# ryogrid/anime-illust-image-searcher

Hardware: AMD Instinct MI355X
Metric: images/sec tagged (ViT fwd) (higher is better)
Workload: dtype f16; 1 GPU; wd-tagger ViT-B/16 448px 16-bit-operand forward + sigmoid + MCut tag selection, batch 64 per GPU, u8 NHWC images resident in HBM (BASELINE.json configs[1]); batch_per_gpu=64, image=448x448x3 u8, classes=10861, parallelism=single GPU

## Files before the change

### anime-illust-image-searcher_amd/csrc/tags.hip

```cpp
#include <vector>

#include "common.h"
#include "rank_util.h"

using namespace hipts;

struct hipts_tagsel {
    int device = 0;
    int C = 0, max_batch = 0;
    int ng = 0, nc = 0, npad = 0;
    DevBuf gidx, cidx;
    DevBuf ws_probs, ws_counts, ws_ids, ws_thresh;
    int ws_row_cap = 0;
};

namespace {

__device__ void bitonic_desc(uint64_t* keys, int npad) {
    for (int size = 2; size <= npad; size <<= 1) {
        for (int stride = size >> 1; stride > 0; stride >>= 1) {
            for (int t = threadIdx.x; t < (npad >> 1); t += blockDim.x) {
                const int lo = ((t / stride) * stride * 2) + (t % stride);
                const int hi = lo + stride;
                const bool desc = ((lo & size) == 0);
                const uint64_t a = keys[lo], b = keys[hi];
                if ((a > b) != desc) {
                    keys[lo] = b;
                    keys[hi] = a;
                }
            }
            __syncthreads();
        }
    }
}

__device__ void select_category(const float* __restrict__ probs, const int32_t* __restrict__ idx, int n, int npad,
                                bool mcut, double thresh_in, bool floor015, uint64_t* keys, double* sh_d, int* sh_i,
                                int32_t* __restrict__ ids_out, int cap, int* count_out, double* thresh_out) {
    const int tid = threadIdx.x, nthr = blockDim.x;
    for (int i = tid; i < npad; i += nthr) {
        uint64_t k = 0;
        if (i < n) k = ((uint64_t)float_order_key_canon(probs[idx[i]]) << 32) | (uint64_t)(0xffffffffu - (uint32_t)i);
        keys[i] = k;
    }
    __syncthreads();
    bitonic_desc(keys, npad);
    double thresh = thresh_in;
    if (mcut && n >= 2) {
        double best = -INFINITY;
        int besti = 0x7fffffff;
        for (int i = tid; i < n - 1; i += nthr) {
            const double a = (double)float_from_key((uint32_t)(keys[i] >> 32));
            const double b = (double)float_from_key((uint32_t)(keys[i + 1] >> 32));
            const double dif = a - b;
            if (dif > best) {
                best = dif;
                besti = i;
            }
        }
        for (int o = 32; o >= 1; o >>= 1) {
            const double ob = __shfl_xor(best, o);
            const int oi = __shfl_xor(besti, o);
            if (ob > best || (ob == best && oi < besti)) {
                best = ob;
                besti = oi;
            }
        }
        if ((tid & 63) == 0) {
            sh_d[tid >> 6] = best;
            sh_i[tid >> 6] = besti;
        }
        __syncthreads();
        if (tid == 0) {
            double b = sh_d[0];
            int bi = sh_i[0];
            for (int w = 1; w < (nthr >> 6); ++w)
                if (sh_d[w] > b || (sh_d[w] == b && sh_i[w] < bi)) {
                    b = sh_d[w];
                    bi = sh_i[w];
                }
            const double a0 = (double)float_from_key((uint32_t)(keys[bi] >> 32));
            const double a1 = (double)float_from_key((uint32_t)(keys[bi + 1] >> 32));
            double t = (a0 + a1) / 2;
            if (floor015 && !(t > 0.15)) t = 0.15;
            sh_d[16] = t;
        }
        __syncthreads();
        thresh = sh_d[16];
        __syncthreads();
    } else if (mcut && floor015 && !(thresh > 0.15)) {
        thresh = 0.15;
    }
    int cnt = 0;
    for (int i = tid; i < n; i += nthr)
        if ((double)float_from_key((uint32_t)(keys[i] >> 32)) > thresh) ++cnt;
    for (int o = 32; o >= 1; o >>= 1) cnt += __shfl_xor(cnt, o);
    if ((tid & 63) == 0) sh_i[tid >> 6] = cnt;
    __syncthreads();
    if (tid == 0) {
        int c = 0;
        for (int w = 0; w < (nthr >> 6); ++w) c += sh_i[w];
        sh_i[16] = c;
    }
    __syncthreads();
    const int total = sh_i[16];
    for (int i = tid; i < total && i < cap; i += nthr)
        ids_out[i] = idx[0xffffffffu - (uint32_t)(keys[i] & 0xffffffffu)];
    if (tid == 0) {
        *count_out = total;
        *thresh_out = thresh;
    }
    __syncthreads();
}

__global__ __launch_bounds__(1024) void tagsel_kernel(const float* __restrict__ probs, int C, const int32_t* __restrict__ gidx,
                                                      int ng, const int32_t* __restrict__ cidx, int nc, int npad,
                                                      double g_thresh, int g_mcut, double c_thresh, int c_mcut,
                                                      int32_t* __restrict__ counts, int counts_stride,
                                                      int32_t* __restrict__ ids, int ids_stride, int row_cap,
                                                      double* __restrict__ thresh) {
    extern __shared__ __attribute__((aligned(16))) uint64_t keys[];
    __shared__ double sh_d[17];
    __shared__ int sh_i[17];
    __shared__ int sh_cnt[2];
    __shared__ double sh_thr[2];
    const int b = blockIdx.x;
    const float* __restrict__ row = probs + (int64_t)b * C;
    int32_t* __restrict__ out = ids + (int64_t)b * ids_stride;
    int npg = 64;
    while (npg < ng) npg <<= 1;
    int npc = 64;
    while (npc < nc) npc <<= 1;
    select_category(row, gidx, ng, npg, g_mcut != 0, g_thresh, false, keys, sh_d, sh_i, out, row_cap, &sh_cnt[0], &sh_thr[0]);
    const int n_g = sh_cnt[0];
    const int used = n_g < row_cap ? n_g : row_cap;
    select_category(row, cidx, nc, npc, c_mcut != 0, c_thresh, true, keys, sh_d, sh_i, out + used, row_cap - used, &sh_cnt[1],
                    &sh_thr[1]);
    if (threadIdx.x == 0) {
        counts[(int64_t)b * counts_stride] = sh_cnt[0];
        counts[(int64_t)b * counts_stride + 1] = sh_cnt[1];
        if (thresh) {
            thresh[2 * b] = sh_thr[0];
            thresh[2 * b + 1] = sh_thr[1];
        }
    }
}

}

extern "C" {

int hipts_tagsel_create(const int32_t* category, int num_classes, int device, int max_batch, hipts_tagsel_t** out) {
    HIPTS_REQUIRE(category && out && num_classes >= 1 && max_batch >= 1, "hipts_tagsel_create: bad arguments");
    HIPTS_TRY(use_device(device));
    std::vector<int32_t> g, c;
    for (int i = 0; i < num_classes; ++i) {
        if (category[i] == 0) g.push_back(i);
        else if (category[i] == 4) c.push_back(i);
    }
    int npad = 64;
    while (npad < (int)g.size() || npad < (int)c.size()) npad <<= 1;
    HIPTS_REQUIRE((size_t)npad * 8 <= 144 * 1024, "hipts_tagsel_create: a category with %zu labels does not fit the LDS sort",
                  g.size() > c.size() ? g.size() : c.size());
    auto* h = new hipts_tagsel();
    h->device = device;
    h->C = num_classes;
    h->max_batch = max_batch;
    h->ng = (int)g.size();
    h->nc = (int)c.size();
    h->npad = npad;
    int st;
    if ((st = h->gidx.alloc(g.size() * 4)) || (st = h->cidx.alloc(c.size() * 4)) || (st = upload(h->gidx.p, g.data(), g.size() * 4)) ||
        (st = upload(h->cidx.p, c.data(), c.size() * 4))) {
        delete h;
        return st;
    }
    hipError_t e = hipFuncSetAttribute((const void*)tagsel_kernel, hipFuncAttributeMaxDynamicSharedMemorySize, 144 * 1024);
    if (e != hipSuccess) {
        delete h;
        return set_error(HIPTS_ERR_HIP, "hipFuncSetAttribute failed: %s", hipGetErrorString(e));
    }
    *out = h;
    return HIPTS_OK;
}

int hipts_tagsel_destroy(hipts_tagsel_t* h) {
    if (h) {
        (void)hipSetDevice(h->device);
        delete h;
    }
    return HIPTS_OK;
}

int hipts_tagsel_run(hipts_tagsel_t* h, const float* probs, int probs_memspace, int batch, double general_thresh,
                     int general_mcut, double character_thresh, int character_mcut, int32_t* counts_out, int32_t* ids_out,
                     int row_cap, double* thresh_out, int out_memspace, void* stream) {
    HIPTS_REQUIRE(h && probs && counts_out && ids_out && batch >= 1 && row_cap >= 1, "hipts_tagsel_run: bad arguments");
    HIPTS_TRY(use_device(h->device));
    hipStream_t s = (hipStream_t)stream;
    const float* p_dev = probs;
    if (probs_memspace != HIPTS_DEVICE) {
        HIPTS_TRY(h->ws_probs.reserve((size_t)batch * h->C * 4));
        HIPTS_HIP(hipMemcpyAsync(h->ws_probs.p, probs, (size_t)batch * h->C * 4, hipMemcpyHostToDevice, s));
        p_dev = h->ws_probs.as<float>();
    }
    int32_t* cnt_dev = counts_out;
    int32_t* ids_dev = ids_out;
    double* thr_dev = thresh_out;
    const bool host_out = out_memspace != HIPTS_DEVICE;
    if (host_out || !thresh_out) {
        HIPTS_TRY(h->ws_thresh.reserve((size_t)batch * 16));
        thr_dev = h->ws_thresh.as<double>();
    }
    if (host_out) {
        HIPTS_TRY(h->ws_counts.reserve((size_t)batch * 8));
        HIPTS_TRY(h->ws_ids.reserve((size_t)batch * row_cap * 4));
        cnt_dev = h->ws_counts.as<int32_t>();
        ids_dev = h->ws_ids.as<int32_t>();
    }
    tagsel_kernel<<<batch, 1024, (size_t)h->npad * 8, s>>>(p_dev, h->C, h->gidx.as<int32_t>(), h->ng, h->cidx.as<int32_t>(), h->nc,
                                                           h->npad, general_thresh, general_mcut, character_thresh,
                                                           character_mcut, cnt_dev, 2, ids_dev, row_cap, row_cap, thr_dev);
    HIPTS_LAUNCH_CHECK();
    if (host_out) {
        HIPTS_HIP(hipMemcpyAsync(counts_out, cnt_dev, (size_t)batch * 8, hipMemcpyDeviceToHost, s));
        HIPTS_HIP(hipMemcpyAsync(ids_out, ids_dev, (size_t)batch * row_cap * 4, hipMemcpyDeviceToHost, s));
        if (thresh_out) HIPTS_HIP(hipMemcpyAsync(thresh_out, thr_dev, (size_t)batch * 16, hipMemcpyDeviceToHost, s));
        HIPTS_HIP(hipStreamSynchronize(s));
    }
    return HIPTS_OK;
}

int hipts_tagsel_run_rows(hipts_tagsel_t* h, const float* probs_device, int batch, double general_thresh, int general_mcut,
                          double character_thresh, int character_mcut, int32_t* rows_device, int row_width, void* stream) {
    HIPTS_REQUIRE(h && probs_device && rows_device && batch >= 1 && row_width >= 3, "hipts_tagsel_run_rows: bad arguments");
    HIPTS_TRY(use_device(h->device));
    tagsel_kernel<<<batch, 1024, (size_t)h->npad * 8, (hipStream_t)stream>>>(
        probs_device, h->C, h->gidx.as<int32_t>(), h->ng, h->cidx.as<int32_t>(), h->nc, h->npad, general_thresh, general_mcut,
        character_thresh, character_mcut, rows_device, row_width, rows_device + 2, row_width, row_width - 2, nullptr);
    HIPTS_LAUNCH_CHECK();
    return HIPTS_OK;
}

}
```

### include/hip_tagsearch_debug.h

```cpp
#ifndef HIP_TAGSEARCH_DEBUG_H
#define HIP_TAGSEARCH_DEBUG_H

#include <stddef.h>
#include <stdint.h>

#include "hip_tagsearch.h"

#ifdef __cplusplus
extern "C" {
#endif

int hiptsdbg_gemm_time(int M, int N, int K, int epi, int iters, float* ms_out);
int hiptsdbg_gemm_clock(int M, int N, int K, int epi, int iters, float* ms_out, float* loop_ghz);
int hiptsdbg_gemm_q4_compare(int M, int N, int K, int epi, int f16, int iters, long long* mismatch_out, float* ms_out);
int hiptsdbg_gelu(const float* x_host, int n, int tanh_form, float* y_host);
int hiptsdbg_dwconv7(const uint16_t* in_f16, const float* w, uint16_t* out_f16, int batch, int H, int C, int mode, int iters, float* ms_out);
int hiptsdbg_dwconv7_stamps(unsigned long long* host, int n);
int hiptsdbg_convnext_stream(hipts_convnext_t* h, const float* x_host, int batch, int stage, float* out_host);
int hiptsdbg_swinv2_stream(hipts_swinv2_t* h, const float* x_host, int batch, int stage, float* out_host);
int hiptsdbg_swinv2_window_attention(const float* q, const float* k, const float* v, const float* logit_scale, const float* cpb, int batch,
                                     int heads, int side, int window, int shift, int operand_f16, float* out);
int hiptsdbg_mlp_fused(const uint16_t* xn, const float* w1, const float* w2, float* x, const float* res_scale, const float* gamma, uint16_t* xn_out,
                       int M, int C, float star_s, float star_b, float eps, int iters, float* ms_out, int waves);
int hiptsdbg_mlp_stamps(unsigned long long* host, int n);
int hiptsdbg_mlp_weight_image(const float* w1, const float* w2, int C, uint16_t* out, long long out_halves);
int hiptsdbg_dw_toeplitz(const float* w, int channels, uint32_t* out);
enum { HIPTSDBG_GEMM_V1 = 0, HIPTSDBG_GEMM_PP = 1, HIPTSDBG_GEMM_S3 = 2, HIPTSDBG_GEMM_PP2 = 3, HIPTSDBG_GEMM_DW = 4,
       HIPTSDBG_GEMM_Q4 = 5, HIPTSDBG_GEMM_PP_E4M3 = 6 };
typedef struct hiptsdbg_gemm_plan_t {
    int32_t loop, mr, interior, stamped;
    int32_t tiles_m, tiles_n, grid, block, lds_bytes;
    int32_t sk_first, sk_slices;
    int32_t raster_gm, raster_gn, epi_prio, epi_prefetch;
    int32_t error;
} hiptsdbg_gemm_plan_t;
int hiptsdbg_gemm_plan(int epi, int M, int N, int K, int f16, int shared_chip, unsigned features, int ld_out, int dim, int cus,
                       unsigned q4_mask, hiptsdbg_gemm_plan_t* out);
int hiptsdbg_gemm_tile_walk(int tiles_m, int tiles_n, int tile_rows, int raster_gm, int raster_gn, int32_t* m0, int32_t* n0);
int hiptsdbg_gemm_kernel_resources(int epi, int mr, int f16, int op8, int sk, int interior, int* num_regs, int* scratch_bytes, int* static_lds);
typedef struct hiptsdbg_gemm_case_t {
    int32_t epi, M, N, K, f16, shared_chip;
    const uint16_t* a;
    const uint16_t* w;
    const float* bias;
    const float* pos;
    const float* res_scale;
    const float* ln_gamma;
    const float* ln_beta;
    const float* col_u;
    const float* rowstat;
    const float* stat_in;
    const float* rope;
    const float* x_init;
    uint64_t x_init_bytes;
    int32_t tokens, tokens_pad, heads, dim, hd_log2;
    int32_t stat_in_blocks, stat_in_stride, ln_dim, rope_tokens, stat_stride;
    int32_t gelu_tanh, star_kind, ld_out, x_blocked, sk_ws, fill;
    float qscale, ln_eps, star_scale, star_bias;
} hiptsdbg_gemm_case_t;
typedef struct hiptsdbg_gemm_out_t {
    void* x;
    void* rowmajor;
    void* probs;
    void* out16[3];
    void* stat_part;
    uint64_t x_bytes, rowmajor_bytes, probs_bytes, out16_bytes[3], stat_part_bytes;
} hiptsdbg_gemm_out_t;
int hiptsdbg_gemm_epilogue(const hiptsdbg_gemm_case_t* in, hiptsdbg_gemm_out_t* out);
enum { HIPTSDBG_SRC_F32 = 0, HIPTSDBG_SRC_F32_BLOCKED = 1, HIPTSDBG_SRC_F32_INPLACE = 2, HIPTSDBG_SRC_16_BIAS = 3 };
enum { HIPTSDBG_AFF_GAMMA_BETA = 0, HIPTSDBG_AFF_GAMMA_OPT_BETA = 1, HIPTSDBG_AFF_GAMMA_ADD_ZERO = 2, HIPTSDBG_AFF_GAMMA_PLAIN = 3 };
enum { HIPTSDBG_SINK_16 = 0, HIPTSDBG_SINK_E4M3 = 1, HIPTSDBG_SINK_F32 = 2, HIPTSDBG_SINK_F32_AND_16 = 3, HIPTSDBG_SINK_PATCH2X2 = 4,
       HIPTSDBG_SINK_ADD_HILO = 5, HIPTSDBG_SINK_BACK = 6 };
typedef struct hiptsdbg_row_ln_case_t {
    int32_t src, affine, sink, f16, blk, H, D, fill;
    int64_t rows;
    float eps;
    const void* in;
    uint64_t in_bytes;
    const float* bias;
    const float* g;
    const float* b;
    const float* x_init;
    uint64_t x_init_bytes;
} hiptsdbg_row_ln_case_t;
typedef struct hiptsdbg_rows_out_t {
    void* f32;
    void* o16;
    uint64_t f32_bytes, o16_bytes;
} hiptsdbg_rows_out_t;
int hiptsdbg_row_ln(const hiptsdbg_row_ln_case_t* in, hiptsdbg_rows_out_t* out);
int hiptsdbg_pool_ln(const float* x, uint64_t x_bytes, const float* g, const float* b, int batch, int T, int C, int count, int blk, float eps,
                     int hilo, int f16, int fill, void* out, uint64_t out_bytes);
int hiptsdbg_rowstat(const float* part, uint64_t part_bytes, int M, int stride, int blocks, int D, float eps, int fill, float* out, uint64_t out_bytes);
int hiptsdbg_fold_ln(const uint16_t* w16, int f16, const float* gamma, const float* beta, const float* bias, int N, int K, int fill, float* u, float* c,
                     uint64_t out_bytes);
enum { HIPTSDBG_PIX_U8_AFFINE = 0, HIPTSDBG_PIX_U8_TABLE = 1, HIPTSDBG_PIX_F32_FLIP = 2, HIPTSDBG_PIX_F32 = 3, HIPTSDBG_PIX_U8_RAW = 4 };
enum { HIPTSDBG_WIN_PATCH = 0, HIPTSDBG_WIN_4X4 = 1, HIPTSDBG_WIN_7X7 = 2 };
int hiptsdbg_patch_gather(int pixel, int window, int f16, const void* images, uint64_t image_bytes, const float* lut, int batch, int S, int P,
                          int KH, int fill, uint16_t* a0, uint64_t a0_bytes);
int hiptsdbg_ccip_stem_u8(const uint8_t* images, const float* lut, int batch, int S, int f16, int fill, uint16_t* a0, uint64_t a0_bytes);
int hiptsdbg_vit_patchify_u8_p16(const uint8_t* images, int batch, int grid, int f16, int fill, uint16_t* a0, uint64_t a0_bytes);
int hiptsdbg_vit_pool(const float* x, uint64_t x_bytes, const float* g, const float* b, int batch, int tokens, int D, float eps, int pool_then_norm,
                      int splits, int f16, int fill, float* part_out, uint64_t part_bytes, uint16_t* out16, uint64_t out16_bytes);
int hiptsdbg_eva_assemble(const float* tmp, uint64_t tmp_bytes, const float* cls, const float* pos, int batch, int np, int TS, int D, int blocked, int fill,
                          float* x, uint64_t x_bytes, float* xblk, uint64_t xblk_bytes);
int hiptsdbg_eva_colsum(const float* x, uint64_t x_bytes, int batch, int np, int TS, int D, int fill, float* part, uint64_t part_bytes);
int hiptsdbg_swinv2_merge(const float* x, uint64_t x_bytes, int batch, int H, int C, int f16, int fill, uint16_t* col, uint64_t col_bytes);
int hiptsdbg_swinv2_split_x(const float* x, uint64_t x_bytes, int64_t rows, int D, int f16, int fill, uint16_t* xh2, uint64_t xh2_bytes);
int hiptsdbg_swinv2_mean(const float* y, uint64_t y_bytes, int batch, int T, int C, int f16, int fill, uint16_t* out, uint64_t out_bytes);
int hiptsdbg_ccip_ds_im2col(const uint16_t* xn, uint64_t xn_bytes, int batch, int H, int C, int fill, uint16_t* col, uint64_t col_bytes);
int hiptsdbg_convnext_cast(const float* x, uint64_t x_bytes, int64_t n4, int f16, int fill, uint16_t* xh, uint64_t xh_bytes);
int hiptsdbg_gemm_run(int M, int N, int K, const uint16_t* a_bf16, const uint16_t* w_bf16, float* out_host);
int hiptsdbg_gemm8_run(int M, int N, int K, const float* a_f32, const float* w_f32, int kind, void* out_host, int* w_exp);
int hiptsdbg_vit_dump(hipts_vit_t* h, const char* name, void* out_host, size_t max_bytes, size_t* bytes);

int hiptsdbg_attention_run(const uint16_t* q, const uint16_t* k, const uint16_t* vT, uint16_t* out_host, int batch, int heads, int tokens,
                           int tokens_pad, int head_dim, int f16);
int hiptsdbg_attention_time(const uint16_t* q, const uint16_t* k, const uint16_t* vT, int batch, int heads, int tokens, int tokens_pad,
                            int head_dim, int f16, int iters, double* avg_us);

int hiptsdbg_attention2(const uint16_t* q, const uint16_t* k, const uint16_t* v, uint16_t* out_host, int batch, int heads, int tokens, int tokens_pad,
                        int f16, int variant, int iters, double* avg_us);

int hiptsdbg_attention2_launch(const uint16_t* q, const uint16_t* k, const uint16_t* v, uint16_t* out_host, long long out_rows, int batch, int heads,
                               int tokens, int tokens_pad, int f16, int out_tokens_stride, int variant, int split_lo);

int hiptsdbg_attention2_kernel_resources(int tokens_pad, int f16, int variant, int* num_regs, int* scratch_bytes, int* static_lds);

int hiptsdbg_attention2_stamps(unsigned long long* host, int n);

int hiptsdbg_search1_last(hipts_bm25_t* h, uint32_t* candidates, uint32_t* took_candidate_path);
enum { HIPTSDBG_QUERY_FINISH = 1, HIPTSDBG_QUERY_WIDE = 2, HIPTSDBG_QUERY_TILED = 4, HIPTSDBG_QUERY_PARTS = 8, HIPTSDBG_QUERY_DEFAULT = 15 };
typedef struct hiptsdbg_search1_plan_t {
    int64_t waves;
    int32_t kk, gw, gl, groups, bcap, finish;
    int32_t grid_score, blocks2, blocks3, reserved;
    uint64_t off_wmax, off_bcnt, off_bflag, off_bkey, off_bid, off_wit, ws_bytes;
    uint64_t out_bytes, off_flag;
} hiptsdbg_search1_plan_t;
int hiptsdbg_search1_plan(int64_t D, int k, unsigned knob_bits, hiptsdbg_search1_plan_t* out);
typedef struct hiptsdbg_sim_plan_t {
    int32_t wide_passes, wide_grid, last_n, last_nqb, last_grid;
    int32_t tail_q0, tail_passes, tail_grid, tail_tiled;
    int32_t parts_grid, index_passes, reserved;
    uint64_t parts_bytes;
} hiptsdbg_sim_plan_t;
int hiptsdbg_sim_plan(int have_tiled, int64_t D, int K, int nq, int want_parts, unsigned knob_bits, hiptsdbg_sim_plan_t* out);
int hiptsdbg_topk_stamps(unsigned long long* host16);
int hiptsdbg_related_last(const hipts_bm25_t* h, double* count_ms, int64_t* lds_items, int64_t* direct_items);
int hiptsdbg_radius_passes(const hipts_radius_t* h, double* pass1_ms, double* pass2_ms, double* sort_ms);

#ifdef __cplusplus
}
#endif
#endif
```

Before: 5621 images/sec.

## Add histogram-pruned fast tag selection pass with full-sort fallback

Adds a 256-thread fast kernel that histograms probability keys per category, keeps only the top few hundred candidates in LDS and bitonic-sorts that small set instead of the whole padded category. It checks that MCut's answer cannot be changed by the pruned tail and flags rows it cannot prove. A gated 1024-thread full-sort kernel then reprocesses only the flagged rows. This cuts sort work and LDS pressure in the post-processing stage, at the cost of an extra kernel launch and a per-row atomic stats counter.

```diff
diff --git a/anime-illust-image-searcher_amd/csrc/tags.hip b/anime-illust-image-searcher_amd/csrc/tags.hip
--- a/anime-illust-image-searcher_amd/csrc/tags.hip
+++ b/anime-illust-image-searcher_amd/csrc/tags.hip
@@ -2,8 +2,13 @@
 
 #include "common.h"
 #include "rank_util.h"
+#include "../../include/hip_tagsearch_debug.h"
 
 using namespace hipts;
+
+#ifndef HIPTS_TAGSEL_CAP
+#define HIPTS_TAGSEL_CAP 512
+#endif
 
 struct hipts_tagsel {
     int device = 0;
@@ -12,9 +17,20 @@
     DevBuf gidx, cidx;
     DevBuf ws_probs, ws_counts, ws_ids, ws_thresh;
     int ws_row_cap = 0;
+    DevBuf flags;
+    DevBuf stats;
+    int path = HIPTSDBG_TAGSEL_AUTO;
 };
 
 namespace {
+
+constexpr int kFastThreads = 256;
+constexpr int kFastCap = HIPTS_TAGSEL_CAP;
+constexpr int kFastBinShift = 21;
+constexpr int kFastBins = 1 << (32 - kFastBinShift);
+constexpr int kFastBinsPerThread = kFastBins / kFastThreads;
+static_assert((kFastCap & (kFastCap - 1)) == 0 && kFastCap >= 64 && kFastCap * 8 + kFastBins * 4 + 1024 <= 32 * 1024,
+              "the fast pass keeps to 32 KB of LDS");
 
 __device__ void bitonic_desc(uint64_t* keys, int npad) {
     for (int size = 2; size <= npad; size <<= 1) {
@@ -34,65 +50,78 @@
     }
 }
 
-__device__ void select_category(const float* __restrict__ probs, const int32_t* __restrict__ idx, int n, int npad,
-                                bool mcut, double thresh_in, bool floor015, uint64_t* keys, double* sh_d, int* sh_i,
-                                int32_t* __restrict__ ids_out, int cap, int* count_out, double* thresh_out) {
+__device__ __forceinline__ uint64_t composite_key(float p, int i) {
+    return ((uint64_t)float_order_key_canon(p) << 32) | (uint64_t)(0xffffffffu - (uint32_t)i);
+}
+
+template <typename F>
+__device__ __forceinline__ void for_each_label(const float* __restrict__ probs, const int32_t* __restrict__ idx, int n, F f) {
+    constexpr int U = 8;
+    for (int i0 = threadIdx.x; i0 < n; i0 += kFastThreads * U) {
+        int32_t id[U];
+        float p[U];
+#pragma unroll
+        for (int u = 0; u < U; ++u) id[u] = i0 + u * kFastThreads < n ? idx[i0 + u * kFastThreads] : 0;
+#pragma unroll
+        for (int u = 0; u < U; ++u) p[u] = i0 + u * kFastThreads < n ? probs[id[u]] : 0.f;
+#pragma unroll
+        for (int u = 0; u < U; ++u)
+            if (i0 + u * kFastThreads < n) f(p[u], i0 + u * kFastThreads);
+    }
+}
+
+__device__ double mcut_threshold(const uint64_t* keys, int ns, bool has_low, uint32_t low_key, bool floor015, double* sh_d, int* sh_i,
+                                 double* gap) {
     const int tid = threadIdx.x, nthr = blockDim.x;
-    for (int i = tid; i < npad; i += nthr) {
-        uint64_t k = 0;
-        if (i < n) k = ((uint64_t)float_order_key_canon(probs[idx[i]]) << 32) | (uint64_t)(0xffffffffu - (uint32_t)i);
-        keys[i] = k;
-    }
-    __syncthreads();
-    bitonic_desc(keys, npad);
-    double thresh = thresh_in;
-    if (mcut && n >= 2) {
-        double best = -INFINITY;
-        int besti = 0x7fffffff;
-        for (int i = tid; i < n - 1; i += nthr) {
-            const double a = (double)float_from_key((uint32_t)(keys[i] >> 32));
-            const double b = (double)float_from_key((uint32_t)(keys[i + 1] >> 32));
-            const double dif = a - b;
-            if (dif > best) {
-                best = dif;
-                besti = i;
+    const int m = ns + (has_low ? 1 : 0);
+    auto value = [&](int i) { return (double)float_from_key(i < ns ? (uint32_t)(keys[i] >> 32) : low_key); };
+    double best = -INFINITY;
+    int besti = 0x7fffffff;
+    for (int i = tid; i < m - 1; i += nthr) {
+        const double dif = value(i) - value(i + 1);
+        if (dif > best) {
+            best = dif;
+            besti = i;
+        }
+    }
+    for (int o = 32; o >= 1; o >>= 1) {
+        const double ob = __shfl_xor(best, o);
+        const int oi = __shfl_xor(besti, o);
+        if (ob > best || (ob == best && oi < besti)) {
+            best = ob;
+            besti = oi;
+        }
+    }
+    if ((tid & 63) == 0) {
+        sh_d[tid >> 6] = best;
+        sh_i[tid >> 6] = besti;
+    }
+    __syncthreads();
+    if (tid == 0) {
+        double b = sh_d[0];
+        int bi = sh_i[0];
+        for (int w = 1; w < (nthr >> 6); ++w)
+            if (sh_d[w] > b || (sh_d[w] == b && sh_i[w] < bi)) {
+                b = sh_d[w];
+                bi = sh_i[w];
             }
-        }
-        for (int o = 32; o >= 1; o >>= 1) {
-            const double ob = __shfl_xor(best, o);
-            const int oi = __shfl_xor(besti, o);
-            if (ob > best || (ob == best && oi < besti)) {
-                best = ob;
-                besti = oi;
-            }
-        }
-        if ((tid & 63) == 0) {
-            sh_d[tid >> 6] = best;
-            sh_i[tid >> 6] = besti;
-        }
-        __syncthreads();
-        if (tid == 0) {
-            double b = sh_d[0];
-            int bi = sh_i[0];
-            for (int w = 1; w < (nthr >> 6); ++w)
-                if (sh_d[w] > b || (sh_d[w] == b && sh_i[w] < bi)) {
-                    b = sh_d[w];
-                    bi = sh_i[w];
-                }
-            const double a0 = (double)float_from_key((uint32_t)(keys[bi] >> 32));
-            const double a1 = (double)float_from_key((uint32_t)(keys[bi + 1] >> 32));
-            double t = (a0 + a1) / 2;
-            if (floor015 && !(t > 0.15)) t = 0.15;
-            sh_d[16] = t;
-        }
-        __syncthreads();
-        thresh = sh_d[16];
-        __syncthreads();
-    } else if (mcut && floor015 && !(thresh > 0.15)) {
-        thresh = 0.15;
-    }
+        double t = (value(bi) + value(bi + 1)) / 2;
+        if (floor015 && !(t > 0.15)) t = 0.15;
+        sh_d[16] = t;
+        sh_d[17] = b;
+    }
+    __syncthreads();
+    const double thresh = sh_d[16];
+    *gap = sh_d[17];
+    __syncthreads();
+    return thresh;
+}
+
+__device__ void emit_prefix(const uint64_t* keys, int ns, double thresh, const int32_t* __restrict__ idx, int* sh_i,
+                            int32_t* __restrict__ ids_out, int cap, int* count_out, double* thresh_out) {
+    const int tid = threadIdx.x, nthr = blockDim.x;
     int cnt = 0;
-    for (int i = tid; i < n; i += nthr)
+    for (int i = tid; i < ns; i += nthr)
         if ((double)float_from_key((uint32_t)(keys[i] >> 32)) > thresh) ++cnt;
     for (int o = 32; o >= 1; o >>= 1) cnt += __shfl_xor(cnt, o);
     if ((tid & 63) == 0) sh_i[tid >> 6] = cnt;
@@ -113,29 +142,150 @@
     __syncthreads();
 }
 
-__global__ __launch_bounds__(1024) void tagsel_kernel(const float* __restrict__ probs, int C, const int32_t* __restrict__ gidx,
-                                                      int ng, const int32_t* __restrict__ cidx, int nc, int npad,
-                                                      double g_thresh, int g_mcut, double c_thresh, int c_mcut,
-                                                      int32_t* __restrict__ counts, int counts_stride,
-                                                      int32_t* __restrict__ ids, int ids_stride, int row_cap,
-                                                      double* __restrict__ thresh) {
+__device__ __forceinline__ double plain_threshold(bool mcut, double thresh_in, bool floor015) {
+    return (mcut && floor015 && !(thresh_in > 0.15)) ? 0.15 : thresh_in;
+}
+
+__device__ void select_category(const float* __restrict__ probs, const int32_t* __restrict__ idx, int n, int npad,
+                                bool mcut, double thresh_in, bool floor015, uint64_t* keys, double* sh_d, int* sh_i,
+                                int32_t* __restrict__ ids_out, int cap, int* count_out, double* thresh_out) {
+    const int tid = threadIdx.x, nthr = blockDim.x;
+    for (int i = tid; i < npad; i += nthr) keys[i] = i < n ? composite_key(probs[idx[i]], i) : 0;
+    __syncthreads();
+    bitonic_desc(keys, npad);
+    double gap;
+    const double thresh = (mcut && n >= 2) ? mcut_threshold(keys, n, false, 0, floor015, sh_d, sh_i, &gap)
+                                           : plain_threshold(mcut, thresh_in, floor015);
+    emit_prefix(keys, n, thresh, idx, sh_i, ids_out, cap, count_out, thresh_out);
+}
+
+__device__ bool select_category_fast(const float* __restrict__ probs, const int32_t* __restrict__ idx, int n, bool mcut,
+                                     double thresh_in, bool floor015, uint64_t* keys, uint32_t* hist, uint32_t* sh_u, double* sh_d,
+                                     int* sh_i, int32_t* __restrict__ ids_out, int cap, int* count_out, double* thresh_out) {
+    enum { FILL = 0, LOW = 1, MIN = 2, BAD = 3, BOUND = 4, NT = 5 };
+    const int tid = threadIdx.x;
+    for (int i = tid; i < kFastBins; i += kFastThreads) hist[i] = 0;
+    if (tid == 0) {
+        sh_u[FILL] = 0;
+        sh_u[LOW] = 0;
+        sh_u[MIN] = 0xffffffffu;
+        sh_u[BAD] = 0;
+        sh_u[BOUND] = 0;
+        sh_u[NT] = (uint32_t)n;
+    }
+    __syncthreads();
+    uint32_t kmin = 0xffffffffu;
+    bool bad = false;
+    for_each_label(probs, idx, n, [&](float p, int) {
+        bad |= !(fabsf(p) <= 3.4028234663852886e38f);
+        const uint32_t k = float_order_key_canon(p);
+        atomicAdd(&hist[k >> kFastBinShift], 1u);
+        kmin = k < kmin ? k : kmin;
+    });
+    if (n > 0 && tid < n) atomicMin(&sh_u[MIN], kmin);
+    if (bad) sh_u[BAD] = 1;
+    __syncthreads();
+    if (sh_u[BAD]) return false;
+    const int top = kFastBins - 1 - kFastBinsPerThread * tid;
+    uint32_t local = 0;
+#pragma unroll
+    for (int j = 0; j < kFastBinsPerThread; ++j) local += hist[top - j];
+    uint32_t incl = local;
+#pragma unroll
+    for (int o = 1; o < 64; o <<= 1) {
+        const uint32_t y = __shfl_up(incl, o);
+        if ((tid & 63) >= o) incl += y;
+    }
+    if ((tid & 63) == 63) sh_i[tid >> 6] = (int)incl;
+    __syncthreads();
+    uint32_t excl = incl - local;
+    for (int w = 0; w < (tid >> 6); ++w) excl += (uint32_t)sh_i[w];
+    if (excl <= (uint32_t)kFastCap && excl + local > (uint32_t)kFastCap) {
+        uint32_t run = excl;
+        for (int j = 0; j < kFastBinsPerThread; ++j) {
+            const uint32_t h = hist[top - j];
+            if (run + h > (uint32_t)kFastCap) {
+                sh_u[BOUND] = (uint32_t)(top - j + 1);
+                sh_u[NT] = run;
+                break;
+            }
+            run += h;
+        }
+    }
+    __syncthreads();
+    const uint32_t bound = sh_u[BOUND];
+    const int nt = (int)sh_u[NT];
+    if (nt == 0 && n > 0) return false;
+    int npt = 2;
+    while (npt < nt) npt <<= 1;
+    uint32_t klow = 0;
+    for_each_label(probs, idx, n, [&](float p, int i) {
+        const uint32_t k = float_order_key_canon(p);
+        if ((k >> kFastBinShift) >= bound) {
+            const uint32_t slot = atomicAdd(&sh_u[FILL], 1u);
+            if (slot < (uint32_t)kFastCap) keys[slot] = composite_key(p, i);
+        } else {
+            klow = k > klow ? k : klow;
+        }
+    });
+    if (klow) atomicMax(&sh_u[LOW], klow);
+    for (int i = nt + tid; i < npt; i += kFastThreads) keys[i] = 0;
+    __syncthreads();
+    if ((int)sh_u[FILL] != nt) return false;
+    bitonic_desc(keys, npt);
+    const bool has_low = nt < n;
+    const uint32_t low_key = sh_u[LOW];
+    double thresh;
+    if (mcut && n >= 2) {
+        double gap;
+        thresh = mcut_threshold(keys, nt, has_low, low_key, floor015, sh_d, sh_i, &gap);
+        if (has_low && !(gap >= (double)float_from_key(low_key) - (double)float_from_key(sh_u[MIN]))) return false;
+    } else {
+        thresh = plain_threshold(mcut, thresh_in, floor015);
+        if (has_low && (double)float_from_key(low_key) > thresh) return false;
+    }
+    emit_prefix(keys, nt, thresh, idx, sh_i, ids_out, cap, count_out, thresh_out);
+    return true;
+}
+
+template <bool FAST>
+__global__ __launch_bounds__(FAST ? kFastThreads : 1024) void tagsel_kernel(
+    const float* __restrict__ probs, int C, const int32_t* __restrict__ gidx, int ng, const int32_t* __restrict__ cidx, int nc, int npad,
+    double g_thresh, int g_mcut, double c_thresh, int c_mcut, int32_t* __restrict__ counts, int counts_stride, int32_t* __restrict__ ids,
+    int ids_stride, int row_cap, double* __restrict__ thresh, int32_t* __restrict__ flags, unsigned long long* __restrict__ stats, int gate) {
     extern __shared__ __attribute__((aligned(16))) uint64_t keys[];
-    __shared__ double sh_d[17];
+    __shared__ double sh_d[18];
     __shared__ int sh_i[17];
     __shared__ int sh_cnt[2];
     __shared__ double sh_thr[2];
     const int b = blockIdx.x;
     const float* __restrict__ row = probs + (int64_t)b * C;
     int32_t* __restrict__ out = ids + (int64_t)b * ids_stride;
-    int npg = 64;
-    while (npg < ng) npg <<= 1;
-    int npc = 64;
-    while (npc < nc) npc <<= 1;
-    select_category(row, gidx, ng, npg, g_mcut != 0, g_thresh, false, keys, sh_d, sh_i, out, row_cap, &sh_cnt[0], &sh_thr[0]);
-    const int n_g = sh_cnt[0];
-    const int used = n_g < row_cap ? n_g : row_cap;
-    select_category(row, cidx, nc, npc, c_mcut != 0, c_thresh, true, keys, sh_d, sh_i, out + used, row_cap - used, &sh_cnt[1],
-                    &sh_thr[1]);
+    if constexpr (FAST) {
+        __shared__ uint32_t hist[kFastBins];
+        __shared__ uint32_t sh_u[6];
+        bool ok = select_category_fast(row, gidx, ng, g_mcut != 0, g_thresh, false, keys, hist, sh_u, sh_d, sh_i, out, row_cap, &sh_cnt[0],
+                                       &sh_thr[0]);
+        if (ok) {
+            const int n_g = sh_cnt[0];
+            const int used = n_g < row_cap ? n_g : row_cap;
+            ok = select_category_fast(row, cidx, nc, c_mcut != 0, c_thresh, true, keys, hist, sh_u, sh_d, sh_i, out + used, row_cap - used,
+                                      &sh_cnt[1], &sh_thr[1]);
+        }
+        if (threadIdx.x == 0) flags[b] = ok ? 0 : 1;
+        if (!ok) return;
+    } else {
+        if (gate && flags[b] == 0) return;
+        int npg = 64;
+        while (npg < ng) npg <<= 1;
+        int npc = 64;
+        while (npc < nc) npc <<= 1;
+        select_category(row, gidx, ng, npg, g_mcut != 0, g_thresh, false, keys, sh_d, sh_i, out, row_cap, &sh_cnt[0], &sh_thr[0]);
+        const int n_g = sh_cnt[0];
+        const int used = n_g < row_cap ? n_g : row_cap;
+        select_category(row, cidx, nc, npc, c_mcut != 0, c_thresh, true, keys, sh_d, sh_i, out + used, row_cap - used, &sh_cnt[1],
+                        &sh_thr[1]);
+    }
     if (threadIdx.x == 0) {
         counts[(int64_t)b * counts_stride] = sh_cnt[0];
         counts[(int64_t)b * counts_stride + 1] = sh_cnt[1];
@@ -143,7 +293,38 @@
             thresh[2 * b] = sh_thr[0];
             thresh[2 * b + 1] = sh_thr[1];
         }
-    }
+        atomicAdd(&stats[FAST ? 0 : 1], 2ull);
+    }
+}
+
+int launch_tagsel(hipts_tagsel* h, const float* probs, int batch, double g_thresh, int g_mcut, double c_thresh, int c_mcut, int32_t* counts,
+                  int counts_stride, int32_t* ids, int ids_stride, int row_cap, double* thresh, hipStream_t s) {
+    HIPTS_TRY(h->flags.reserve((size_t)batch * 4));
+    int32_t* flags = h->flags.as<int32_t>();
+    unsigned long long* stats = h->stats.as<unsigned long long>();
+    const int32_t *gidx = h->gidx.as<int32_t>(), *cidx = h->cidx.as<int32_t>();
+    if (h->path != HIPTSDBG_TAGSEL_FULL) {
+        tagsel_kernel<true><<<batch, kFastThreads, (size_t)kFastCap * 8, s>>>(probs, h->C, gidx, h->ng, cidx, h->nc, h->npad, g_thresh, g_mcut,
+                                                                               c_thresh, c_mcut, counts, counts_stride, ids, ids_stride,
+                                                                               row_cap, thresh, flags, stats, 0);
+        HIPTS_LAUNCH_CHECK();
+    }
+    if (h->path != HIPTSDBG_TAGSEL_FAST_ONLY) {
+        tagsel_kernel<false><<<batch, 1024, (size_t)h->npad * 8, s>>>(probs, h->C, gidx, h->ng, cidx, h->nc, h->npad, g_thresh, g_mcut,
+                                                                       c_thresh, c_mcut, counts, counts_stride, ids, ids_stride, row_cap,
+                                                                       thresh, flags, stats, h->path == HIPTSDBG_TAGSEL_AUTO ? 1 : 0);
+        HIPTS_LAUNCH_CHECK();
+        return HIPTS_OK;
+    }
+    std::vector<int32_t> host((size_t)batch);
+    HIPTS_HIP(hipMemcpyAsync(host.data(), flags, (size_t)batch * 4, hipMemcpyDeviceToHost, s));
+    HIPTS_HIP(hipStreamSynchronize(s));
+    int left = 0;
+    for (int32_t f : host) left += f != 0;
+    if (left)
+        return set_error(HIPTS_ERR_STATE, "tag selection: the fast pass could not finish %d of %d images and the full path is switched off",
+                         left, batch);
+    return HIPTS_OK;
 }
 
 }
@@ -171,14 +352,15 @@
     h->npad = npad;
     int st;
     if ((st = h->gidx.alloc(g.size() * 4)) || (st = h->cidx.alloc(c.size() * 4)) || (st = upload(h->gidx.p, g.data(), g.size() * 4)) ||
-        (st = upload(h->cidx.p, c.data(), c.size() * 4))) {
+        (st = upload(h->cidx.p, c.data(), c.size() * 4)) || (st = h->flags.alloc((size_t)max_batch * 4)) || (st = h->stats.alloc(16))) {
         delete h;
         return st;
     }
-    hipError_t e = hipFuncSetAttribute((const void*)tagsel_kernel, hipFuncAttributeMaxDynamicSharedMemorySize, 144 * 1024);
+    hipError_t e = hipMemset(h->stats.p, 0, 16);
+    if (e == hipSuccess) e = hipFuncSetAttribute((const void*)tagsel_kernel<false>, hipFuncAttributeMaxDynamicSharedMemorySize, 144 * 1024);
     if (e != hipSuccess) {
         delete h;
-        return set_error(HIPTS_ERR_HIP, "hipFuncSetAttribute failed: %s", hipGetErrorString(e));
+        return set_error(HIPTS_ERR_HIP, "hipMemset / hipFuncSetAttribute failed: %s", hipGetErrorString(e));
     }
     *out = h;
     return HIPTS_OK;
@@ -218,10 +400,8 @@
         cnt_dev = h->ws_counts.as<int32_t>();
         ids_dev = h->ws_ids.as<int32_t>();
     }
-    tagsel_kernel<<<batch, 1024, (size_t)h->npad * 8, s>>>(p_dev, h->C, h->gidx.as<int32_t>(), h->ng, h->cidx.as<int32_t>(), h->nc,
-                                                           h->npad, general_thresh, general_mcut, character_thresh,
-                                                           character_mcut, cnt_dev, 2, ids_dev, row_cap, row_cap, thr_dev);
-    HIPTS_LAUNCH_CHECK();
+    HIPTS_TRY(launch_tagsel(h, p_dev, batch, general_thresh, general_mcut, character_thresh, character_mcut, cnt_dev, 2, ids_dev, row_cap,
+                            row_cap, thr_dev, s));
     if (host_out) {
         HIPTS_HIP(hipMemcpyAsync(counts_out, cnt_dev, (size_t)batch * 8, hipMemcpyDeviceToHost, s));
         HIPTS_HIP(hipMemcpyAsync(ids_out, ids_dev, (size_t)batch * row_cap * 4, hipMemcpyDeviceToHost, s));
@@ -235,11 +415,36 @@
                           double character_thresh, int character_mcut, int32_t* rows_device, int row_width, void* stream) {
     HIPTS_REQUIRE(h && probs_device && rows_device && batch >= 1 && row_width >= 3, "hipts_tagsel_run_rows: bad arguments");
     HIPTS_TRY(use_device(h->device));
-    tagsel_kernel<<<batch, 1024, (size_t)h->npad * 8, (hipStream_t)stream>>>(
-        probs_device, h->C, h->gidx.as<int32_t>(), h->ng, h->cidx.as<int32_t>(), h->nc, h->npad, general_thresh, general_mcut,
-        character_thresh, character_mcut, rows_device, row_width, rows_device + 2, row_width, row_width - 2, nullptr);
-    HIPTS_LAUNCH_CHECK();
-    return HIPTS_OK;
-}
-
-}
+    return launch_tagsel(h, probs_device, batch, general_thresh, general_mcut, character_thresh, character_mcut, rows_device, row_width,
+                         rows_device + 2, row_width, row_width - 2, nullptr, (hipStream_t)stream);
+}
+
+int hiptsdbg_tagsel_set_path(hipts_tagsel_t* h, int path) {
+    HIPTS_REQUIRE(h && path >= HIPTSDBG_TAGSEL_AUTO && path <= HIPTSDBG_TAGSEL_FULL, "hiptsdbg_tagsel_set_path: bad arguments");
+    h->path = path;
+    return HIPTS_OK;
+}
+
+int hiptsdbg_tagsel_counters(hipts_tagsel_t* h, int64_t* fast_categories, int64_t* full_categories) {
+    HIPTS_REQUIRE(h, "hiptsdbg_tagsel_counters: bad arguments");
+    HIPTS_TRY(use_device(h->device));
+    unsigned long long v[2];
+    HIPTS_HIP(hipDeviceSynchronize());
+    HIPTS_HIP(hipMemcpy(v, h->stats.p, 16, hipMemcpyDeviceToHost));
+    if (fast_categories) *fast_categories = (int64_t)v[0];
+    if (full_categories) *full_categories = (int64_t)v[1];
+    return HIPTS_OK;
+}
+
+int hiptsdbg_tagsel_kernel_resources(int fast, int* max_threads, int* static_lds, int* dynamic_lds, int* cap) {
+    HIPTS_REQUIRE(max_threads && static_lds && dynamic_lds && cap, "hiptsdbg_tagsel_kernel_resources: bad arguments");
+    hipFuncAttributes a;
+    HIPTS_HIP(hipFuncGetAttributes(&a, fast ? (const void*)tagsel_kernel<true> : (const void*)tagsel_kernel<false>));
+    *max_threads = a.maxThreadsPerBlock;
+    *static_lds = (int)a.sharedSizeBytes;
+    *dynamic_lds = fast ? kFastCap * 8 : 0;
+    *cap = kFastCap;
+    return HIPTS_OK;
+}
+
+}
diff --git a/include/hip_tagsearch_debug.h b/include/hip_tagsearch_debug.h
--- a/include/hip_tagsearch_debug.h
+++ b/include/hip_tagsearch_debug.h
@@ -150,6 +150,11 @@
 int hiptsdbg_related_last(const hipts_bm25_t* h, double* count_ms, int64_t* lds_items, int64_t* direct_items);
 int hiptsdbg_radius_passes(const hipts_radius_t* h, double* pass1_ms, double* pass2_ms, double* sort_ms);
 
+enum { HIPTSDBG_TAGSEL_AUTO = 0, HIPTSDBG_TAGSEL_FAST_ONLY = 1, HIPTSDBG_TAGSEL_FULL = 2 };
+int hiptsdbg_tagsel_set_path(hipts_tagsel_t* h, int path);
+int hiptsdbg_tagsel_counters(hipts_tagsel_t* h, int64_t* fast_categories, int64_t* full_categories);
+int hiptsdbg_tagsel_kernel_resources(int fast, int* max_threads, int* static_lds, int* dynamic_lds, int* cap);
+
 #ifdef __cplusplus
 }
 #endif
```

Result: no change. 5641 images/sec, median of 6 (+0.4%).
